# Boese0601/MagicDance

Hardware: NVIDIA H100
Metric: denoise-steps/sec @512x512 50-step DDIM (higher is better)
Workload: dtype f16

## Files before the change

### magicdance_b200/csrc/attention.cu

```cuda
#include <stdlib.h>

#include <type_traits>

#include "common.cuh"

namespace mdb {

constexpr int kBQ = 128;

template <int D, int BKV, int STAGES>
struct AttnCfg {
  static constexpr int kDkChunks = (D + 63) / 64;
  static constexpr int kDV = (D + 15) / 16 * 16;
  static constexpr int kKSteps = kDV / 16;
  static constexpr int kQBytes = kDkChunks * kBQ * 128;
  static constexpr int kKBytes = kDkChunks * BKV * 128;
  static constexpr int kVBytes = kDV * 128;
  static constexpr int kStageBytes = kKBytes + kVBytes;
  static constexpr int kSmem = kQBytes + STAGES * kStageBytes + 1024;
  static_assert(BKV == 64, "one 128-byte swizzle row of keys per V^T tile");
  static_assert(kVBytes % 1024 == 0 && kKBytes % 1024 == 0, "stage tiles start on swizzle-atom boundaries");
};

struct AttnKParams {
  CUtensorMap tmQ, tmK0, tmV0, tmK1, tmV1;
  __half* out;
  long long ldo;
  int nq, n0, n1;
  int kv0_batches, kv1_batches;
  int bank_batches;
  float scale_log2;
};
struct AttnLseKParams : AttnKParams {
  float* lse;
};

template <int D, int BKV, int STAGES, int MINB, bool LSE = false>
__global__ void __launch_bounds__(kWsThreads, MINB)
    attn_wg_kernel(const __grid_constant__ std::conditional_t<LSE, AttnLseKParams, AttnKParams> p) {
  using C = AttnCfg<D, BKV, STAGES>;
  extern __shared__ uint8_t smem_raw[];
  __shared__ __align__(8) uint64_t q_bar;
  __shared__ __align__(8) uint64_t kv_full[STAGES], kv_empty[STAGES];

  uint8_t* sQ = align1024(smem_raw);
  uint8_t* sKV = sQ + C::kQBytes;

  const int warp = threadIdx.x >> 5;
  const int lane = threadIdx.x & 31;
  const int q0 = blockIdx.x * kBQ;
  const int head = blockIdx.y;
  const int b = blockIdx.z;
  const int t0 = (p.n0 + BKV - 1) / BKV;
  const int t1 = (b < p.bank_batches && p.n1 > 0) ? (p.n1 + BKV - 1) / BKV : 0;
  const int n_tiles = t0 + t1;

  pdl_launch_dependents();
  if (warp == kProducerWarp && lane == 0) {
    tma_prefetch_desc(&p.tmQ);
    tma_prefetch_desc(&p.tmK0);
    tma_prefetch_desc(&p.tmV0);
    mbar_init(&q_bar, 1);
    ring_init<STAGES>(kv_full, kv_empty, 1);
    fence_barrier_init();
  }
  __syncthreads();
  pdl_wait();

  if (warp == kProducerWarp) {
    if (lane == 0) {
      mbar_expect_tx(&q_bar, C::kQBytes);
      for (int dc = 0; dc < C::kDkChunks; ++dc)
        tma_load_3d(sQ + dc * (kBQ * 128), &p.tmQ, &q_bar, dc * 64, head, b * p.nq + q0);
      for (int j = 0; j < n_tiles; ++j) {
        const bool src1 = j >= t0;
        const int key0 = (src1 ? (j - t0) : j) * BKV;
        const CUtensorMap* tk = src1 ? &p.tmK1 : &p.tmK0;
        const CUtensorMap* tv = src1 ? &p.tmV1 : &p.tmV0;
        const int nsrc = src1 ? p.n1 : p.n0;
        const int kvb = src1 ? (p.kv1_batches > 1 ? b : 0) : (p.kv0_batches > 1 ? b : 0);
        const int s = ring_acquire<STAGES>(kv_empty, j);
        mbar_expect_tx(&kv_full[s], C::kStageBytes);
        uint8_t* sk = sKV + s * C::kStageBytes;
        uint8_t* sv = sk + C::kKBytes;
        for (int dc = 0; dc < C::kDkChunks; ++dc)
          tma_load_3d(sk + dc * (BKV * 128), tk, &kv_full[s], dc * 64, head, kvb * nsrc + key0);
        tma_load_3d(sv, tv, &kv_full[s], key0, kvb, head * D);
      }
    }
  } else {
    const int wg = warp >> 2;
    const uint32_t q_addr = smem_u32(sQ) + wg * (64 * 128);
    const int cq = 2 * (lane & 3);
    float o[C::kDV / 2];
#pragma unroll
    for (int i = 0; i < C::kDV / 2; ++i) o[i] = 0.f;
    float m_run[2] = {-INFINITY, -INFINITY};
    float l_run[2] = {0.f, 0.f};
    mbar_wait(&q_bar, 0);

    for (int j = 0; j < n_tiles; ++j) {
      const bool src1 = j >= t0;
      const int key0 = (src1 ? (j - t0) : j) * BKV;
      const int valid = min(BKV, (src1 ? p.n1 : p.n0) - key0);
      const int s = ring_wait_full<STAGES>(kv_full, j);
      const uint32_t k_addr = smem_u32(sKV + s * C::kStageBytes);
      const uint32_t v_addr = k_addr + C::kKBytes;

      float sc[BKV / 2];
      wgmma_fence();
#pragma unroll
      for (int ks = 0; ks < C::kKSteps; ++ks) {
        const int dc = ks >> 2, kk = ks & 3;
        const uint64_t da = wgmma_desc_k_sw128(q_addr + dc * (kBQ * 128)) + 2 * kk;
        const uint64_t db = wgmma_desc_k_sw128(k_addr + dc * (BKV * 128)) + 2 * kk;
        wgmma_ss<BKV>(sc, da, db, ks != 0 ? 1u : 0u);
      }
      wgmma_commit();
      wgmma_wait<0>();
      wgmma_fence_regs(sc);

      if (valid < BKV) {
#pragma unroll
        for (int i = 0; i < BKV / 2; ++i)
          if (8 * (i >> 2) + cq + (i & 1) >= valid) sc[i] = -INFINITY;
      }
      float mx[2] = {-INFINITY, -INFINITY};
#pragma unroll
      for (int i = 0; i < BKV / 2; ++i) mx[(i >> 1) & 1] = fmaxf(mx[(i >> 1) & 1], sc[i]);
      float alpha[2], neg_m[2];
#pragma unroll
      for (int h = 0; h < 2; ++h) {
        mx[h] = fmaxf(mx[h], __shfl_xor_sync(0xffffffffu, mx[h], 1));
        mx[h] = fmaxf(mx[h], __shfl_xor_sync(0xffffffffu, mx[h], 2));
        const float m_new = fmaxf(m_run[h], mx[h] * p.scale_log2);
        alpha[h] = ex2_approx(m_run[h] - m_new);
        m_run[h] = m_new;
        neg_m[h] = -m_new;
      }
      float ls[2] = {0.f, 0.f};
      uint32_t pa[BKV / 16][4];
#pragma unroll
      for (int i = 0; i < BKV / 2; i += 2) {
        const int h = (i >> 1) & 1;
        const float e0 = ex2_approx(fmaf(sc[i], p.scale_log2, neg_m[h]));
        const float e1 = ex2_approx(fmaf(sc[i + 1], p.scale_log2, neg_m[h]));
        ls[h] += e0 + e1;
        pa[i >> 3][(i >> 1) & 3] = pack_half2(e0, e1);
      }
#pragma unroll
      for (int h = 0; h < 2; ++h) l_run[h] = fmaf(l_run[h], alpha[h], ls[h]);
#pragma unroll
      for (int i = 0; i < C::kDV / 2; ++i) o[i] *= alpha[(i >> 1) & 1];

      wgmma_fence();
#pragma unroll
      for (int kk = 0; kk < BKV / 16; ++kk)
        wgmma_rs<C::kDV>(o, pa[kk], wgmma_desc_k_sw128(v_addr) + 2 * kk, 1u);
      wgmma_commit();
      wgmma_wait<0>();
      wgmma_fence_regs(o);
      mbar_arrive(&kv_empty[s]);
    }

    float inv_l[2], l_row[2];
#pragma unroll
    for (int h = 0; h < 2; ++h) {
      float l = l_run[h];
      l += __shfl_xor_sync(0xffffffffu, l, 1);
      l += __shfl_xor_sync(0xffffffffu, l, 2);
      inv_l[h] = 1.0f / l;
      l_row[h] = l;
    }
    const int r = wg * 64 + (warp & 3) * 16 + (lane >> 2);
    if constexpr (LSE) {
      if ((lane & 3) == 0) {
#pragma unroll
        for (int h = 0; h < 2; ++h) {
          const int q = q0 + r + 8 * h;
          if (q < p.nq)
            p.lse[(static_cast<long long>(b) * gridDim.y + head) * p.nq + q] =
                (m_run[h] + log2f(l_row[h])) * 0.6931471805599453f;
        }
      }
    }
#pragma unroll
    for (int h = 0; h < 2; ++h) {
      const int q = q0 + r + 8 * h;
      if (q < p.nq) {
        __half* op = p.out + (static_cast<long long>(b) * p.nq + q) * p.ldo + head * D + cq;
#pragma unroll
        for (int c8 = 0; c8 < D / 8; ++c8)
          *reinterpret_cast<uint32_t*>(op + 8 * c8) =
              pack_half2(o[4 * c8 + 2 * h] * inv_l[h], o[4 * c8 + 2 * h + 1] * inv_l[h]);
      }
    }
  }
}

static int g_attn40_2q_min_ctas = 512;
int get_attn_tuning() { return g_attn40_2q_min_ctas; }
void set_attn_tuning(int v) { g_attn40_2q_min_ctas = v; }

template <int D, int BKV, int STAGES, int MINB, bool LSE = false, typename P>
static int launch_attn(const P& kp, dim3 grid, cudaStream_t st) {
  using C = AttnCfg<D, BKV, STAGES>;
  static_assert(MINB == 1 || C::kSmem <= 113 * 1024, "two CTAs per SM must fit");
  constexpr auto kern = attn_wg_kernel<D, BKV, STAGES, MINB, LSE>;
  if (int rc = set_max_dyn_smem<kern>(C::kSmem)) return rc;
  MDB_CHECK_CUDA(launch_pdl(kern, grid, dim3(kWsThreads), C::kSmem, st, kp));
  count_launch();
  return MDB_OK;
}

template <int D, int BKV>
static int build_and_launch(const mdb_attn_desc* a, float* lse, cudaStream_t st) {
  constexpr int kDV = AttnCfg<D, BKV, 1>::kDV;
  AttnKParams kp;
  memset(&kp, 0, sizeof(kp));
  const int hd = a->heads * a->d;
  int rc;
  if ((rc = tmap_heads(&kp.tmQ, a->q, a->d, a->heads, (uint64_t)a->batch * a->nq, a->ldq, kBQ))) return rc;
  auto mk_kv = [&](const void* k, long long ldk, const void* vt, long long ldvt, int n, int nb, int ldvb,
                   CUtensorMap* tk, CUtensorMap* tv) -> int {
    int r = tmap_heads(tk, k, a->d, a->heads, (uint64_t)nb * n, ldk, BKV);
    if (r) return r;
    return tmap_vt(tv, vt, n, nb, ldvb, hd, ldvt, kDV);
  };
  if ((rc = mk_kv(a->k0, a->ldk0, a->vt0, a->ldvt0, a->n0, a->kv0_batches, a->ldv0_batch, &kp.tmK0, &kp.tmV0))) return rc;
  if (a->n1 > 0) {
    if ((rc = mk_kv(a->k1, a->ldk1, a->vt1, a->ldvt1, a->n1, a->kv1_batches, a->ldv1_batch, &kp.tmK1, &kp.tmV1)))
      return rc;
  }
  kp.out = static_cast<__half*>(a->out);
  kp.ldo = a->ldo;
  kp.nq = a->nq;
  kp.n0 = a->n0;
  kp.n1 = a->n1;
  kp.kv0_batches = a->kv0_batches;
  kp.kv1_batches = a->kv1_batches;
  kp.bank_batches = a->n1 > 0 ? a->bank_batches : 0;
  kp.scale_log2 = a->scale * 1.4426950408889634f;
  dim3 grid((a->nq + kBQ - 1) / kBQ, a->heads, a->batch);
  if (lse != nullptr) {
    AttnLseKParams lp;
    memset(&lp, 0, sizeof(lp));
    static_cast<AttnKParams&>(lp) = kp;
    lp.lse = lse;
    if constexpr (D == 40) {
      const long long ctas = (long long)grid.x * grid.y * grid.z;
      if (ctas >= (long long)g_attn40_2q_min_ctas) return launch_attn<D, BKV, 3, 2, true>(lp, grid, st);
    }
    return launch_attn<D, BKV, (D == 160 ? 2 : 4), 1, true>(lp, grid, st);
  }
  if constexpr (D == 40) {
    const long long ctas = (long long)grid.x * grid.y * grid.z;
    if (ctas >= (long long)g_attn40_2q_min_ctas) return launch_attn<D, BKV, 3, 2>(kp, grid, st);
  }
  return launch_attn<D, BKV, (D == 160 ? 2 : 4), 1>(kp, grid, st);
}

static int attention_entry(const mdb_attn_desc* a, float* lse, cudaStream_t st) {
  switch (a->d) {
    case 40:
      return build_and_launch<40, 64>(a, lse, st);
    case 80:
      return build_and_launch<80, 64>(a, lse, st);
    case 160:
      return build_and_launch<160, 64>(a, lse, st);
    default:
      set_error("mdb_attention_f16: head dim %d not supported (40, 80, 160)", a->d);
      return MDB_ERR_UNSUPPORTED;
  }
}

int attention_check_desc(const mdb_attn_desc* a) {
  MDB_REQUIRE(a != nullptr, "mdb_attention_f16: null descriptor");
  MDB_REQUIRE(a->q && a->k0 && a->vt0 && a->out, "mdb_attention_f16: null operand");
  MDB_REQUIRE(a->batch > 0 && a->heads > 0 && a->nq > 0 && a->n0 > 0 && a->n1 >= 0,
              "mdb_attention_f16: bad shape");
  MDB_REQUIRE(a->n1 == 0 || (a->k1 && a->vt1), "mdb_attention_f16: n1 > 0 needs k1/vt1");
  MDB_REQUIRE(a->kv0_batches == 1 || a->kv0_batches == a->batch, "mdb_attention_f16: kv0_batches must be 1 or batch");
  MDB_REQUIRE(a->n1 == 0 || a->kv1_batches == 1 || a->kv1_batches >= a->bank_batches,
              "mdb_attention_f16: kv1_batches must be 1 or cover bank_batches");
  MDB_REQUIRE(a->ldv0_batch >= a->n0 && a->ldv0_batch % 8 == 0, "mdb_attention_f16: ldv0_batch must be >= n0 and %% 8");
  MDB_REQUIRE(a->n1 == 0 || (a->ldv1_batch >= a->n1 && a->ldv1_batch % 8 == 0),
              "mdb_attention_f16: ldv1_batch must be >= n1 and %% 8");
  MDB_REQUIRE(a->ldo % 8 == 0 && (reinterpret_cast<uintptr_t>(a->out) & 15) == 0, "mdb_attention_f16: out alignment");
  return MDB_OK;
}

}

using namespace mdb;

extern "C" int mdb_attention_f16(const mdb_attn_desc* a, mdb_stream_t stream) {
  const int rc = attention_check_desc(a);
  if (rc) return rc;
  return attention_entry(a, nullptr, static_cast<cudaStream_t>(stream));
}

extern "C" int mdb_attention_lse_f16(const mdb_attn_desc* a, float* lse, mdb_stream_t stream) {
  const int rc = attention_check_desc(a);
  if (rc) return rc;
  MDB_REQUIRE(lse != nullptr, "mdb_attention_lse_f16: null lse");
  return attention_entry(a, lse, static_cast<cudaStream_t>(stream));
}
```

### magicdance_b200/csrc/wgmma.cuh

```cuda
#pragma once
#include <stdint.h>

namespace mdb {

template <int N, int TA = 0, int TB = 0>
__device__ __forceinline__ void wgmma_ss(float (&d)[N / 2], uint64_t da, uint64_t db, uint32_t acc);
template <int N, int TB = 0>
__device__ __forceinline__ void wgmma_rs(float (&d)[N / 2], const uint32_t (&a)[4], uint64_t db, uint32_t acc);

template <>
__device__ __forceinline__ void wgmma_ss<64, 0, 0>(float (&d)[32], uint64_t da, uint64_t db, uint32_t acc) {
  asm volatile(
      "{\n\t.reg .pred p;\n\tsetp.ne.b32 p, %34, 0;\n\t"
      "wgmma.mma_async.sync.aligned.m64n64k16.f32.f16.f16 {%0, %1, %2, %3, %4, %5, %6, %7, %8, %9, %10, %11, %12, %13, %14, %15, %16, %17, %18, %19, %20, %21, %22, %23, %24, %25, %26, %27, %28, %29, %30, %31}, %32, %33, p, 1, 1, 0, 0;\n\t}"
      : "+f"(d[0]), "+f"(d[1]), "+f"(d[2]), "+f"(d[3]), "+f"(d[4]), "+f"(d[5]), "+f"(d[6]), "+f"(d[7]), "+f"(d[8]), "+f"(d[9]), "+f"(d[10]), "+f"(d[11]), "+f"(d[12]), "+f"(d[13]), "+f"(d[14]), "+f"(d[15]), "+f"(d[16]), "+f"(d[17]), "+f"(d[18]), "+f"(d[19]), "+f"(d[20]), "+f"(d[21]), "+f"(d[22]), "+f"(d[23]), "+f"(d[24]), "+f"(d[25]), "+f"(d[26]), "+f"(d[27]), "+f"(d[28]), "+f"(d[29]), "+f"(d[30]), "+f"(d[31])
      : "l"(da), "l"(db), "r"(acc));
}

template <>
__device__ __forceinline__ void wgmma_ss<80, 0, 0>(float (&d)[40], uint64_t da, uint64_t db, uint32_t acc) {
  asm volatile(
      "{\n\t.reg .pred p;\n\tsetp.ne.b32 p, %42, 0;\n\t"
      "wgmma.mma_async.sync.aligned.m64n80k16.f32.f16.f16 {%0, %1, %2, %3, %4, %5, %6, %7, %8, %9, %10, %11, %12, %13, %14, %15, %16, %17, %18, %19, %20, %21, %22, %23, %24, %25, %26, %27, %28, %29, %30, %31, %32, %33, %34, %35, %36, %37, %38, %39}, %40, %41, p, 1, 1, 0, 0;\n\t}"
      : "+f"(d[0]), "+f"(d[1]), "+f"(d[2]), "+f"(d[3]), "+f"(d[4]), "+f"(d[5]), "+f"(d[6]), "+f"(d[7]), "+f"(d[8]), "+f"(d[9]), "+f"(d[10]), "+f"(d[11]), "+f"(d[12]), "+f"(d[13]), "+f"(d[14]), "+f"(d[15]), "+f"(d[16]), "+f"(d[17]), "+f"(d[18]), "+f"(d[19]), "+f"(d[20]), "+f"(d[21]), "+f"(d[22]), "+f"(d[23]), "+f"(d[24]), "+f"(d[25]), "+f"(d[26]), "+f"(d[27]), "+f"(d[28]), "+f"(d[29]), "+f"(d[30]), "+f"(d[31]), "+f"(d[32]), "+f"(d[33]), "+f"(d[34]), "+f"(d[35]), "+f"(d[36]), "+f"(d[37]), "+f"(d[38]), "+f"(d[39])
      : "l"(da), "l"(db), "r"(acc));
}

template <>
__device__ __forceinline__ void wgmma_ss<128, 0, 0>(float (&d)[64], uint64_t da, uint64_t db, uint32_t acc) {
  asm volatile(
      "{\n\t.reg .pred p;\n\tsetp.ne.b32 p, %66, 0;\n\t"
      "wgmma.mma_async.sync.aligned.m64n128k16.f32.f16.f16 {%0, %1, %2, %3, %4, %5, %6, %7, %8, %9, %10, %11, %12, %13, %14, %15, %16, %17, %18, %19, %20, %21, %22, %23, %24, %25, %26, %27, %28, %29, %30, %31, %32, %33, %34, %35, %36, %37, %38, %39, %40, %41, %42, %43, %44, %45, %46, %47, %48, %49, %50, %51, %52, %53, %54, %55, %56, %57, %58, %59, %60, %61, %62, %63}, %64, %65, p, 1, 1, 0, 0;\n\t}"
      : "+f"(d[0]), "+f"(d[1]), "+f"(d[2]), "+f"(d[3]), "+f"(d[4]), "+f"(d[5]), "+f"(d[6]), "+f"(d[7]), "+f"(d[8]), "+f"(d[9]), "+f"(d[10]), "+f"(d[11]), "+f"(d[12]), "+f"(d[13]), "+f"(d[14]), "+f"(d[15]), "+f"(d[16]), "+f"(d[17]), "+f"(d[18]), "+f"(d[19]), "+f"(d[20]), "+f"(d[21]), "+f"(d[22]), "+f"(d[23]), "+f"(d[24]), "+f"(d[25]), "+f"(d[26]), "+f"(d[27]), "+f"(d[28]), "+f"(d[29]), "+f"(d[30]), "+f"(d[31]), "+f"(d[32]), "+f"(d[33]), "+f"(d[34]), "+f"(d[35]), "+f"(d[36]), "+f"(d[37]), "+f"(d[38]), "+f"(d[39]), "+f"(d[40]), "+f"(d[41]), "+f"(d[42]), "+f"(d[43]), "+f"(d[44]), "+f"(d[45]), "+f"(d[46]), "+f"(d[47]), "+f"(d[48]), "+f"(d[49]), "+f"(d[50]), "+f"(d[51]), "+f"(d[52]), "+f"(d[53]), "+f"(d[54]), "+f"(d[55]), "+f"(d[56]), "+f"(d[57]), "+f"(d[58]), "+f"(d[59]), "+f"(d[60]), "+f"(d[61]), "+f"(d[62]), "+f"(d[63])
      : "l"(da), "l"(db), "r"(acc));
}

template <>
__device__ __forceinline__ void wgmma_ss<160, 0, 0>(float (&d)[80], uint64_t da, uint64_t db, uint32_t acc) {
  asm volatile(
      "{\n\t.reg .pred p;\n\tsetp.ne.b32 p, %82, 0;\n\t"
      "wgmma.mma_async.sync.aligned.m64n160k16.f32.f16.f16 {%0, %1, %2, %3, %4, %5, %6, %7, %8, %9, %10, %11, %12, %13, %14, %15, %16, %17, %18, %19, %20, %21, %22, %23, %24, %25, %26, %27, %28, %29, %30, %31, %32, %33, %34, %35, %36, %37, %38, %39, %40, %41, %42, %43, %44, %45, %46, %47, %48, %49, %50, %51, %52, %53, %54, %55, %56, %57, %58, %59, %60, %61, %62, %63, %64, %65, %66, %67, %68, %69, %70, %71, %72, %73, %74, %75, %76, %77, %78, %79}, %80, %81, p, 1, 1, 0, 0;\n\t}"
      : "+f"(d[0]), "+f"(d[1]), "+f"(d[2]), "+f"(d[3]), "+f"(d[4]), "+f"(d[5]), "+f"(d[6]), "+f"(d[7]), "+f"(d[8]), "+f"(d[9]), "+f"(d[10]), "+f"(d[11]), "+f"(d[12]), "+f"(d[13]), "+f"(d[14]), "+f"(d[15]), "+f"(d[16]), "+f"(d[17]), "+f"(d[18]), "+f"(d[19]), "+f"(d[20]), "+f"(d[21]), "+f"(d[22]), "+f"(d[23]), "+f"(d[24]), "+f"(d[25]), "+f"(d[26]), "+f"(d[27]), "+f"(d[28]), "+f"(d[29]), "+f"(d[30]), "+f"(d[31]), "+f"(d[32]), "+f"(d[33]), "+f"(d[34]), "+f"(d[35]), "+f"(d[36]), "+f"(d[37]), "+f"(d[38]), "+f"(d[39]), "+f"(d[40]), "+f"(d[41]), "+f"(d[42]), "+f"(d[43]), "+f"(d[44]), "+f"(d[45]), "+f"(d[46]), "+f"(d[47]), "+f"(d[48]), "+f"(d[49]), "+f"(d[50]), "+f"(d[51]), "+f"(d[52]), "+f"(d[53]), "+f"(d[54]), "+f"(d[55]), "+f"(d[56]), "+f"(d[57]), "+f"(d[58]), "+f"(d[59]), "+f"(d[60]), "+f"(d[61]), "+f"(d[62]), "+f"(d[63]), "+f"(d[64]), "+f"(d[65]), "+f"(d[66]), "+f"(d[67]), "+f"(d[68]), "+f"(d[69]), "+f"(d[70]), "+f"(d[71]), "+f"(d[72]), "+f"(d[73]), "+f"(d[74]), "+f"(d[75]), "+f"(d[76]), "+f"(d[77]), "+f"(d[78]), "+f"(d[79])
      : "l"(da), "l"(db), "r"(acc));
}

template <>
__device__ __forceinline__ void wgmma_ss<256, 0, 0>(float (&d)[128], uint64_t da, uint64_t db, uint32_t acc) {
  asm volatile(
      "{\n\t.reg .pred p;\n\tsetp.ne.b32 p, %130, 0;\n\t"
      "wgmma.mma_async.sync.aligned.m64n256k16.f32.f16.f16 {%0, %1, %2, %3, %4, %5, %6, %7, %8, %9, %10, %11, %12, %13, %14, %15, %16, %17, %18, %19, %20, %21, %22, %23, %24, %25, %26, %27, %28, %29, %30, %31, %32, %33, %34, %35, %36, %37, %38, %39, %40, %41, %42, %43, %44, %45, %46, %47, %48, %49, %50, %51, %52, %53, %54, %55, %56, %57, %58, %59, %60, %61, %62, %63, %64, %65, %66, %67, %68, %69, %70, %71, %72, %73, %74, %75, %76, %77, %78, %79, %80, %81, %82, %83, %84, %85, %86, %87, %88, %89, %90, %91, %92, %93, %94, %95, %96, %97, %98, %99, %100, %101, %102, %103, %104, %105, %106, %107, %108, %109, %110, %111, %112, %113, %114, %115, %116, %117, %118, %119, %120, %121, %122, %123, %124, %125, %126, %127}, %128, %129, p, 1, 1, 0, 0;\n\t}"
      : "+f"(d[0]), "+f"(d[1]), "+f"(d[2]), "+f"(d[3]), "+f"(d[4]), "+f"(d[5]), "+f"(d[6]), "+f"(d[7]), "+f"(d[8]), "+f"(d[9]), "+f"(d[10]), "+f"(d[11]), "+f"(d[12]), "+f"(d[13]), "+f"(d[14]), "+f"(d[15]), "+f"(d[16]), "+f"(d[17]), "+f"(d[18]), "+f"(d[19]), "+f"(d[20]), "+f"(d[21]), "+f"(d[22]), "+f"(d[23]), "+f"(d[24]), "+f"(d[25]), "+f"(d[26]), "+f"(d[27]), "+f"(d[28]), "+f"(d[29]), "+f"(d[30]), "+f"(d[31]), "+f"(d[32]), "+f"(d[33]), "+f"(d[34]), "+f"(d[35]), "+f"(d[36]), "+f"(d[37]), "+f"(d[38]), "+f"(d[39]), "+f"(d[40]), "+f"(d[41]), "+f"(d[42]), "+f"(d[43]), "+f"(d[44]), "+f"(d[45]), "+f"(d[46]), "+f"(d[47]), "+f"(d[48]), "+f"(d[49]), "+f"(d[50]), "+f"(d[51]), "+f"(d[52]), "+f"(d[53]), "+f"(d[54]), "+f"(d[55]), "+f"(d[56]), "+f"(d[57]), "+f"(d[58]), "+f"(d[59]), "+f"(d[60]), "+f"(d[61]), "+f"(d[62]), "+f"(d[63]), "+f"(d[64]), "+f"(d[65]), "+f"(d[66]), "+f"(d[67]), "+f"(d[68]), "+f"(d[69]), "+f"(d[70]), "+f"(d[71]), "+f"(d[72]), "+f"(d[73]), "+f"(d[74]), "+f"(d[75]), "+f"(d[76]), "+f"(d[77]), "+f"(d[78]), "+f"(d[79]), "+f"(d[80]), "+f"(d[81]), "+f"(d[82]), "+f"(d[83]), "+f"(d[84]), "+f"(d[85]), "+f"(d[86]), "+f"(d[87]), "+f"(d[88]), "+f"(d[89]), "+f"(d[90]), "+f"(d[91]), "+f"(d[92]), "+f"(d[93]), "+f"(d[94]), "+f"(d[95]), "+f"(d[96]), "+f"(d[97]), "+f"(d[98]), "+f"(d[99]), "+f"(d[100]), "+f"(d[101]), "+f"(d[102]), "+f"(d[103]), "+f"(d[104]), "+f"(d[105]), "+f"(d[106]), "+f"(d[107]), "+f"(d[108]), "+f"(d[109]), "+f"(d[110]), "+f"(d[111]), "+f"(d[112]), "+f"(d[113]), "+f"(d[114]), "+f"(d[115]), "+f"(d[116]), "+f"(d[117]), "+f"(d[118]), "+f"(d[119]), "+f"(d[120]), "+f"(d[121]), "+f"(d[122]), "+f"(d[123]), "+f"(d[124]), "+f"(d[125]), "+f"(d[126]), "+f"(d[127])
      : "l"(da), "l"(db), "r"(acc));
}

template <>
__device__ __forceinline__ void wgmma_ss<64, 0, 1>(float (&d)[32], uint64_t da, uint64_t db, uint32_t acc) {
  asm volatile(
      "{\n\t.reg .pred p;\n\tsetp.ne.b32 p, %34, 0;\n\t"
      "wgmma.mma_async.sync.aligned.m64n64k16.f32.f16.f16 {%0, %1, %2, %3, %4, %5, %6, %7, %8, %9, %10, %11, %12, %13, %14, %15, %16, %17, %18, %19, %20, %21, %22, %23, %24, %25, %26, %27, %28, %29, %30, %31}, %32, %33, p, 1, 1, 0, 1;\n\t}"
      : "+f"(d[0]), "+f"(d[1]), "+f"(d[2]), "+f"(d[3]), "+f"(d[4]), "+f"(d[5]), "+f"(d[6]), "+f"(d[7]), "+f"(d[8]), "+f"(d[9]), "+f"(d[10]), "+f"(d[11]), "+f"(d[12]), "+f"(d[13]), "+f"(d[14]), "+f"(d[15]), "+f"(d[16]), "+f"(d[17]), "+f"(d[18]), "+f"(d[19]), "+f"(d[20]), "+f"(d[21]), "+f"(d[22]), "+f"(d[23]), "+f"(d[24]), "+f"(d[25]), "+f"(d[26]), "+f"(d[27]), "+f"(d[28]), "+f"(d[29]), "+f"(d[30]), "+f"(d[31])
      : "l"(da), "l"(db), "r"(acc));
}

template <>
__device__ __forceinline__ void wgmma_ss<64, 1, 0>(float (&d)[32], uint64_t da, uint64_t db, uint32_t acc) {
  asm volatile(
      "{\n\t.reg .pred p;\n\tsetp.ne.b32 p, %34, 0;\n\t"
      "wgmma.mma_async.sync.aligned.m64n64k16.f32.f16.f16 {%0, %1, %2, %3, %4, %5, %6, %7, %8, %9, %10, %11, %12, %13, %14, %15, %16, %17, %18, %19, %20, %21, %22, %23, %24, %25, %26, %27, %28, %29, %30, %31}, %32, %33, p, 1, 1, 1, 0;\n\t}"
      : "+f"(d[0]), "+f"(d[1]), "+f"(d[2]), "+f"(d[3]), "+f"(d[4]), "+f"(d[5]), "+f"(d[6]), "+f"(d[7]), "+f"(d[8]), "+f"(d[9]), "+f"(d[10]), "+f"(d[11]), "+f"(d[12]), "+f"(d[13]), "+f"(d[14]), "+f"(d[15]), "+f"(d[16]), "+f"(d[17]), "+f"(d[18]), "+f"(d[19]), "+f"(d[20]), "+f"(d[21]), "+f"(d[22]), "+f"(d[23]), "+f"(d[24]), "+f"(d[25]), "+f"(d[26]), "+f"(d[27]), "+f"(d[28]), "+f"(d[29]), "+f"(d[30]), "+f"(d[31])
      : "l"(da), "l"(db), "r"(acc));
}

template <>
__device__ __forceinline__ void wgmma_ss<128, 0, 1>(float (&d)[64], uint64_t da, uint64_t db, uint32_t acc) {
  asm volatile(
      "{\n\t.reg .pred p;\n\tsetp.ne.b32 p, %66, 0;\n\t"
      "wgmma.mma_async.sync.aligned.m64n128k16.f32.f16.f16 {%0, %1, %2, %3, %4, %5, %6, %7, %8, %9, %10, %11, %12, %13, %14, %15, %16, %17, %18, %19, %20, %21, %22, %23, %24, %25, %26, %27, %28, %29, %30, %31, %32, %33, %34, %35, %36, %37, %38, %39, %40, %41, %42, %43, %44, %45, %46, %47, %48, %49, %50, %51, %52, %53, %54, %55, %56, %57, %58, %59, %60, %61, %62, %63}, %64, %65, p, 1, 1, 0, 1;\n\t}"
      : "+f"(d[0]), "+f"(d[1]), "+f"(d[2]), "+f"(d[3]), "+f"(d[4]), "+f"(d[5]), "+f"(d[6]), "+f"(d[7]), "+f"(d[8]), "+f"(d[9]), "+f"(d[10]), "+f"(d[11]), "+f"(d[12]), "+f"(d[13]), "+f"(d[14]), "+f"(d[15]), "+f"(d[16]), "+f"(d[17]), "+f"(d[18]), "+f"(d[19]), "+f"(d[20]), "+f"(d[21]), "+f"(d[22]), "+f"(d[23]), "+f"(d[24]), "+f"(d[25]), "+f"(d[26]), "+f"(d[27]), "+f"(d[28]), "+f"(d[29]), "+f"(d[30]), "+f"(d[31]), "+f"(d[32]), "+f"(d[33]), "+f"(d[34]), "+f"(d[35]), "+f"(d[36]), "+f"(d[37]), "+f"(d[38]), "+f"(d[39]), "+f"(d[40]), "+f"(d[41]), "+f"(d[42]), "+f"(d[43]), "+f"(d[44]), "+f"(d[45]), "+f"(d[46]), "+f"(d[47]), "+f"(d[48]), "+f"(d[49]), "+f"(d[50]), "+f"(d[51]), "+f"(d[52]), "+f"(d[53]), "+f"(d[54]), "+f"(d[55]), "+f"(d[56]), "+f"(d[57]), "+f"(d[58]), "+f"(d[59]), "+f"(d[60]), "+f"(d[61]), "+f"(d[62]), "+f"(d[63])
      : "l"(da), "l"(db), "r"(acc));
}

template <>
__device__ __forceinline__ void wgmma_ss<128, 1, 1>(float (&d)[64], uint64_t da, uint64_t db, uint32_t acc) {
  asm volatile(
      "{\n\t.reg .pred p;\n\tsetp.ne.b32 p, %66, 0;\n\t"
      "wgmma.mma_async.sync.aligned.m64n128k16.f32.f16.f16 {%0, %1, %2, %3, %4, %5, %6, %7, %8, %9, %10, %11, %12, %13, %14, %15, %16, %17, %18, %19, %20, %21, %22, %23, %24, %25, %26, %27, %28, %29, %30, %31, %32, %33, %34, %35, %36, %37, %38, %39, %40, %41, %42, %43, %44, %45, %46, %47, %48, %49, %50, %51, %52, %53, %54, %55, %56, %57, %58, %59, %60, %61, %62, %63}, %64, %65, p, 1, 1, 1, 1;\n\t}"
      : "+f"(d[0]), "+f"(d[1]), "+f"(d[2]), "+f"(d[3]), "+f"(d[4]), "+f"(d[5]), "+f"(d[6]), "+f"(d[7]), "+f"(d[8]), "+f"(d[9]), "+f"(d[10]), "+f"(d[11]), "+f"(d[12]), "+f"(d[13]), "+f"(d[14]), "+f"(d[15]), "+f"(d[16]), "+f"(d[17]), "+f"(d[18]), "+f"(d[19]), "+f"(d[20]), "+f"(d[21]), "+f"(d[22]), "+f"(d[23]), "+f"(d[24]), "+f"(d[25]), "+f"(d[26]), "+f"(d[27]), "+f"(d[28]), "+f"(d[29]), "+f"(d[30]), "+f"(d[31]), "+f"(d[32]), "+f"(d[33]), "+f"(d[34]), "+f"(d[35]), "+f"(d[36]), "+f"(d[37]), "+f"(d[38]), "+f"(d[39]), "+f"(d[40]), "+f"(d[41]), "+f"(d[42]), "+f"(d[43]), "+f"(d[44]), "+f"(d[45]), "+f"(d[46]), "+f"(d[47]), "+f"(d[48]), "+f"(d[49]), "+f"(d[50]), "+f"(d[51]), "+f"(d[52]), "+f"(d[53]), "+f"(d[54]), "+f"(d[55]), "+f"(d[56]), "+f"(d[57]), "+f"(d[58]), "+f"(d[59]), "+f"(d[60]), "+f"(d[61]), "+f"(d[62]), "+f"(d[63])
      : "l"(da), "l"(db), "r"(acc));
}

template <>
__device__ __forceinline__ void wgmma_rs<48, 0>(float (&d)[24], const uint32_t (&a)[4], uint64_t db, uint32_t acc) {
  asm volatile(
      "{\n\t.reg .pred p;\n\tsetp.ne.b32 p, %29, 0;\n\t"
      "wgmma.mma_async.sync.aligned.m64n48k16.f32.f16.f16 {%0, %1, %2, %3, %4, %5, %6, %7, %8, %9, %10, %11, %12, %13, %14, %15, %16, %17, %18, %19, %20, %21, %22, %23}, {%24, %25, %26, %27}, %28, p, 1, 1, 0;\n\t}"
      : "+f"(d[0]), "+f"(d[1]), "+f"(d[2]), "+f"(d[3]), "+f"(d[4]), "+f"(d[5]), "+f"(d[6]), "+f"(d[7]), "+f"(d[8]), "+f"(d[9]), "+f"(d[10]), "+f"(d[11]), "+f"(d[12]), "+f"(d[13]), "+f"(d[14]), "+f"(d[15]), "+f"(d[16]), "+f"(d[17]), "+f"(d[18]), "+f"(d[19]), "+f"(d[20]), "+f"(d[21]), "+f"(d[22]), "+f"(d[23])
      : "r"(a[0]), "r"(a[1]), "r"(a[2]), "r"(a[3]), "l"(db), "r"(acc));
}

template <>
__device__ __forceinline__ void wgmma_rs<80, 0>(float (&d)[40], const uint32_t (&a)[4], uint64_t db, uint32_t acc) {
  asm volatile(
      "{\n\t.reg .pred p;\n\tsetp.ne.b32 p, %45, 0;\n\t"
      "wgmma.mma_async.sync.aligned.m64n80k16.f32.f16.f16 {%0, %1, %2, %3, %4, %5, %6, %7, %8, %9, %10, %11, %12, %13, %14, %15, %16, %17, %18, %19, %20, %21, %22, %23, %24, %25, %26, %27, %28, %29, %30, %31, %32, %33, %34, %35, %36, %37, %38, %39}, {%40, %41, %42, %43}, %44, p, 1, 1, 0;\n\t}"
      : "+f"(d[0]), "+f"(d[1]), "+f"(d[2]), "+f"(d[3]), "+f"(d[4]), "+f"(d[5]), "+f"(d[6]), "+f"(d[7]), "+f"(d[8]), "+f"(d[9]), "+f"(d[10]), "+f"(d[11]), "+f"(d[12]), "+f"(d[13]), "+f"(d[14]), "+f"(d[15]), "+f"(d[16]), "+f"(d[17]), "+f"(d[18]), "+f"(d[19]), "+f"(d[20]), "+f"(d[21]), "+f"(d[22]), "+f"(d[23]), "+f"(d[24]), "+f"(d[25]), "+f"(d[26]), "+f"(d[27]), "+f"(d[28]), "+f"(d[29]), "+f"(d[30]), "+f"(d[31]), "+f"(d[32]), "+f"(d[33]), "+f"(d[34]), "+f"(d[35]), "+f"(d[36]), "+f"(d[37]), "+f"(d[38]), "+f"(d[39])
      : "r"(a[0]), "r"(a[1]), "r"(a[2]), "r"(a[3]), "l"(db), "r"(acc));
}

template <>
__device__ __forceinline__ void wgmma_rs<160, 0>(float (&d)[80], const uint32_t (&a)[4], uint64_t db, uint32_t acc) {
  asm volatile(
      "{\n\t.reg .pred p;\n\tsetp.ne.b32 p, %85, 0;\n\t"
      "wgmma.mma_async.sync.aligned.m64n160k16.f32.f16.f16 {%0, %1, %2, %3, %4, %5, %6, %7, %8, %9, %10, %11, %12, %13, %14, %15, %16, %17, %18, %19, %20, %21, %22, %23, %24, %25, %26, %27, %28, %29, %30, %31, %32, %33, %34, %35, %36, %37, %38, %39, %40, %41, %42, %43, %44, %45, %46, %47, %48, %49, %50, %51, %52, %53, %54, %55, %56, %57, %58, %59, %60, %61, %62, %63, %64, %65, %66, %67, %68, %69, %70, %71, %72, %73, %74, %75, %76, %77, %78, %79}, {%80, %81, %82, %83}, %84, p, 1, 1, 0;\n\t}"
      : "+f"(d[0]), "+f"(d[1]), "+f"(d[2]), "+f"(d[3]), "+f"(d[4]), "+f"(d[5]), "+f"(d[6]), "+f"(d[7]), "+f"(d[8]), "+f"(d[9]), "+f"(d[10]), "+f"(d[11]), "+f"(d[12]), "+f"(d[13]), "+f"(d[14]), "+f"(d[15]), "+f"(d[16]), "+f"(d[17]), "+f"(d[18]), "+f"(d[19]), "+f"(d[20]), "+f"(d[21]), "+f"(d[22]), "+f"(d[23]), "+f"(d[24]), "+f"(d[25]), "+f"(d[26]), "+f"(d[27]), "+f"(d[28]), "+f"(d[29]), "+f"(d[30]), "+f"(d[31]), "+f"(d[32]), "+f"(d[33]), "+f"(d[34]), "+f"(d[35]), "+f"(d[36]), "+f"(d[37]), "+f"(d[38]), "+f"(d[39]), "+f"(d[40]), "+f"(d[41]), "+f"(d[42]), "+f"(d[43]), "+f"(d[44]), "+f"(d[45]), "+f"(d[46]), "+f"(d[47]), "+f"(d[48]), "+f"(d[49]), "+f"(d[50]), "+f"(d[51]), "+f"(d[52]), "+f"(d[53]), "+f"(d[54]), "+f"(d[55]), "+f"(d[56]), "+f"(d[57]), "+f"(d[58]), "+f"(d[59]), "+f"(d[60]), "+f"(d[61]), "+f"(d[62]), "+f"(d[63]), "+f"(d[64]), "+f"(d[65]), "+f"(d[66]), "+f"(d[67]), "+f"(d[68]), "+f"(d[69]), "+f"(d[70]), "+f"(d[71]), "+f"(d[72]), "+f"(d[73]), "+f"(d[74]), "+f"(d[75]), "+f"(d[76]), "+f"(d[77]), "+f"(d[78]), "+f"(d[79])
      : "r"(a[0]), "r"(a[1]), "r"(a[2]), "r"(a[3]), "l"(db), "r"(acc));
}

template <>
__device__ __forceinline__ void wgmma_rs<48, 1>(float (&d)[24], const uint32_t (&a)[4], uint64_t db, uint32_t acc) {
  asm volatile(
      "{\n\t.reg .pred p;\n\tsetp.ne.b32 p, %29, 0;\n\t"
      "wgmma.mma_async.sync.aligned.m64n48k16.f32.f16.f16 {%0, %1, %2, %3, %4, %5, %6, %7, %8, %9, %10, %11, %12, %13, %14, %15, %16, %17, %18, %19, %20, %21, %22, %23}, {%24, %25, %26, %27}, %28, p, 1, 1, 1;\n\t}"
      : "+f"(d[0]), "+f"(d[1]), "+f"(d[2]), "+f"(d[3]), "+f"(d[4]), "+f"(d[5]), "+f"(d[6]), "+f"(d[7]), "+f"(d[8]), "+f"(d[9]), "+f"(d[10]), "+f"(d[11]), "+f"(d[12]), "+f"(d[13]), "+f"(d[14]), "+f"(d[15]), "+f"(d[16]), "+f"(d[17]), "+f"(d[18]), "+f"(d[19]), "+f"(d[20]), "+f"(d[21]), "+f"(d[22]), "+f"(d[23])
      : "r"(a[0]), "r"(a[1]), "r"(a[2]), "r"(a[3]), "l"(db), "r"(acc));
}

template <>
__device__ __forceinline__ void wgmma_rs<80, 1>(float (&d)[40], const uint32_t (&a)[4], uint64_t db, uint32_t acc) {
  asm volatile(
      "{\n\t.reg .pred p;\n\tsetp.ne.b32 p, %45, 0;\n\t"
      "wgmma.mma_async.sync.aligned.m64n80k16.f32.f16.f16 {%0, %1, %2, %3, %4, %5, %6, %7, %8, %9, %10, %11, %12, %13, %14, %15, %16, %17, %18, %19, %20, %21, %22, %23, %24, %25, %26, %27, %28, %29, %30, %31, %32, %33, %34, %35, %36, %37, %38, %39}, {%40, %41, %42, %43}, %44, p, 1, 1, 1;\n\t}"
      : "+f"(d[0]), "+f"(d[1]), "+f"(d[2]), "+f"(d[3]), "+f"(d[4]), "+f"(d[5]), "+f"(d[6]), "+f"(d[7]), "+f"(d[8]), "+f"(d[9]), "+f"(d[10]), "+f"(d[11]), "+f"(d[12]), "+f"(d[13]), "+f"(d[14]), "+f"(d[15]), "+f"(d[16]), "+f"(d[17]), "+f"(d[18]), "+f"(d[19]), "+f"(d[20]), "+f"(d[21]), "+f"(d[22]), "+f"(d[23]), "+f"(d[24]), "+f"(d[25]), "+f"(d[26]), "+f"(d[27]), "+f"(d[28]), "+f"(d[29]), "+f"(d[30]), "+f"(d[31]), "+f"(d[32]), "+f"(d[33]), "+f"(d[34]), "+f"(d[35]), "+f"(d[36]), "+f"(d[37]), "+f"(d[38]), "+f"(d[39])
      : "r"(a[0]), "r"(a[1]), "r"(a[2]), "r"(a[3]), "l"(db), "r"(acc));
}

template <>
__device__ __forceinline__ void wgmma_rs<160, 1>(float (&d)[80], const uint32_t (&a)[4], uint64_t db, uint32_t acc) {
  asm volatile(
      "{\n\t.reg .pred p;\n\tsetp.ne.b32 p, %85, 0;\n\t"
      "wgmma.mma_async.sync.aligned.m64n160k16.f32.f16.f16 {%0, %1, %2, %3, %4, %5, %6, %7, %8, %9, %10, %11, %12, %13, %14, %15, %16, %17, %18, %19, %20, %21, %22, %23, %24, %25, %26, %27, %28, %29, %30, %31, %32, %33, %34, %35, %36, %37, %38, %39, %40, %41, %42, %43, %44, %45, %46, %47, %48, %49, %50, %51, %52, %53, %54, %55, %56, %57, %58, %59, %60, %61, %62, %63, %64, %65, %66, %67, %68, %69, %70, %71, %72, %73, %74, %75, %76, %77, %78, %79}, {%80, %81, %82, %83}, %84, p, 1, 1, 1;\n\t}"
      : "+f"(d[0]), "+f"(d[1]), "+f"(d[2]), "+f"(d[3]), "+f"(d[4]), "+f"(d[5]), "+f"(d[6]), "+f"(d[7]), "+f"(d[8]), "+f"(d[9]), "+f"(d[10]), "+f"(d[11]), "+f"(d[12]), "+f"(d[13]), "+f"(d[14]), "+f"(d[15]), "+f"(d[16]), "+f"(d[17]), "+f"(d[18]), "+f"(d[19]), "+f"(d[20]), "+f"(d[21]), "+f"(d[22]), "+f"(d[23]), "+f"(d[24]), "+f"(d[25]), "+f"(d[26]), "+f"(d[27]), "+f"(d[28]), "+f"(d[29]), "+f"(d[30]), "+f"(d[31]), "+f"(d[32]), "+f"(d[33]), "+f"(d[34]), "+f"(d[35]), "+f"(d[36]), "+f"(d[37]), "+f"(d[38]), "+f"(d[39]), "+f"(d[40]), "+f"(d[41]), "+f"(d[42]), "+f"(d[43]), "+f"(d[44]), "+f"(d[45]), "+f"(d[46]), "+f"(d[47]), "+f"(d[48]), "+f"(d[49]), "+f"(d[50]), "+f"(d[51]), "+f"(d[52]), "+f"(d[53]), "+f"(d[54]), "+f"(d[55]), "+f"(d[56]), "+f"(d[57]), "+f"(d[58]), "+f"(d[59]), "+f"(d[60]), "+f"(d[61]), "+f"(d[62]), "+f"(d[63]), "+f"(d[64]), "+f"(d[65]), "+f"(d[66]), "+f"(d[67]), "+f"(d[68]), "+f"(d[69]), "+f"(d[70]), "+f"(d[71]), "+f"(d[72]), "+f"(d[73]), "+f"(d[74]), "+f"(d[75]), "+f"(d[76]), "+f"(d[77]), "+f"(d[78]), "+f"(d[79])
      : "r"(a[0]), "r"(a[1]), "r"(a[2]), "r"(a[3]), "l"(db), "r"(acc));
}

}
```

Measured before the change: 89.85.

## Overlap next-tile QK wgmma with current PV wgmma and softmax in attention

Restructures the attention consumer loop into a software pipeline. The QK^T wgmma for the next KV tile is issued together with the PV wgmma for the current tile, and softmax on the new scores runs while PV is still in flight. This hides tensor-core latency behind softmax math. It also narrows the PV N dimension to a multiple of 8 (adding an m64n40 instruction for D=40), which drops padded columns. The pipelined path is enabled for all head sizes except 160, and it keeps more registers live per thread.

```diff
diff --git a/magicdance_b200/csrc/attention.cu b/magicdance_b200/csrc/attention.cu
--- a/magicdance_b200/csrc/attention.cu
+++ b/magicdance_b200/csrc/attention.cu
@@ -12,6 +12,7 @@
 struct AttnCfg {
   static constexpr int kDkChunks = (D + 63) / 64;
   static constexpr int kDV = (D + 15) / 16 * 16;
+  static constexpr int kPvN = (D + 7) / 8 * 8;
   static constexpr int kKSteps = kDV / 16;
   static constexpr int kQBytes = kDkChunks * kBQ * 128;
   static constexpr int kKBytes = kDkChunks * BKV * 128;
@@ -35,7 +36,71 @@
   float* lse;
 };
 
-template <int D, int BKV, int STAGES, int MINB, bool LSE = false>
+template <int D, int BKV>
+__device__ __forceinline__ void attn_issue_qk(float (&sc)[BKV / 2], uint32_t q_addr, uint32_t k_addr) {
+  using C = AttnCfg<D, BKV, 1>;
+  wgmma_fence();
+#pragma unroll
+  for (int ks = 0; ks < C::kKSteps; ++ks) {
+    const int dc = ks >> 2, kk = ks & 3;
+    const uint64_t da = wgmma_desc_k_sw128(q_addr + dc * (kBQ * 128)) + 2 * kk;
+    const uint64_t db = wgmma_desc_k_sw128(k_addr + dc * (BKV * 128)) + 2 * kk;
+    wgmma_ss<BKV>(sc, da, db, ks != 0 ? 1u : 0u);
+  }
+  wgmma_commit();
+}
+
+template <int BKV>
+__device__ __forceinline__ void attn_softmax(float (&sc)[BKV / 2], int valid, float scale_log2, float (&m_run)[2],
+                                             float (&l_run)[2], float (&alpha)[2]) {
+  const int cq = 2 * (threadIdx.x & 3);
+  if (valid < BKV) {
+#pragma unroll
+    for (int i = 0; i < BKV / 2; ++i)
+      if (8 * (i >> 2) + cq + (i & 1) >= valid) sc[i] = -INFINITY;
+  }
+  float mx[2] = {-INFINITY, -INFINITY};
+#pragma unroll
+  for (int i = 0; i < BKV / 2; ++i) mx[(i >> 1) & 1] = fmaxf(mx[(i >> 1) & 1], sc[i]);
+  float neg_m[2];
+#pragma unroll
+  for (int h = 0; h < 2; ++h) {
+    mx[h] = fmaxf(mx[h], __shfl_xor_sync(0xffffffffu, mx[h], 1));
+    mx[h] = fmaxf(mx[h], __shfl_xor_sync(0xffffffffu, mx[h], 2));
+    const float m_new = fmaxf(m_run[h], mx[h] * scale_log2);
+    alpha[h] = ex2_approx(m_run[h] - m_new);
+    m_run[h] = m_new;
+    neg_m[h] = -m_new;
+  }
+  float ls[2] = {0.f, 0.f};
+#pragma unroll
+  for (int i = 0; i < BKV / 2; i += 2) {
+    const int h = (i >> 1) & 1;
+    sc[i] = ex2_approx(fmaf(sc[i], scale_log2, neg_m[h]));
+    sc[i + 1] = ex2_approx(fmaf(sc[i + 1], scale_log2, neg_m[h]));
+    ls[h] += sc[i] + sc[i + 1];
+  }
+#pragma unroll
+  for (int h = 0; h < 2; ++h) l_run[h] = fmaf(l_run[h], alpha[h], ls[h]);
+}
+
+template <int BKV>
+__device__ __forceinline__ void attn_pack_p(const float (&sc)[BKV / 2], uint32_t (&pa)[BKV / 16][4]) {
+#pragma unroll
+  for (int i = 0; i < BKV / 2; i += 2) pa[i >> 3][(i >> 1) & 3] = pack_half2(sc[i], sc[i + 1]);
+}
+
+template <int D, int BKV>
+__device__ __forceinline__ void attn_issue_pv(float (&o)[AttnCfg<D, BKV, 1>::kPvN / 2],
+                                              const uint32_t (&pa)[BKV / 16][4], uint32_t v_addr) {
+  wgmma_fence();
+#pragma unroll
+  for (int kk = 0; kk < BKV / 16; ++kk)
+    wgmma_rs<AttnCfg<D, BKV, 1>::kPvN>(o, pa[kk], wgmma_desc_k_sw128(v_addr) + 2 * kk, 1u);
+  wgmma_commit();
+}
+
+template <int D, int BKV, int STAGES, int MINB, bool PIPE, bool LSE = false>
 __global__ void __launch_bounds__(kWsThreads, MINB)
     attn_wg_kernel(const __grid_constant__ std::conditional_t<LSE, AttnLseKParams, AttnKParams> p) {
   using C = AttnCfg<D, BKV, STAGES>;
@@ -92,75 +157,63 @@
     const int wg = warp >> 2;
     const uint32_t q_addr = smem_u32(sQ) + wg * (64 * 128);
     const int cq = 2 * (lane & 3);
-    float o[C::kDV / 2];
-#pragma unroll
-    for (int i = 0; i < C::kDV / 2; ++i) o[i] = 0.f;
+    float o[C::kPvN / 2];
+#pragma unroll
+    for (int i = 0; i < C::kPvN / 2; ++i) o[i] = 0.f;
     float m_run[2] = {-INFINITY, -INFINITY};
     float l_run[2] = {0.f, 0.f};
     mbar_wait(&q_bar, 0);
 
-    for (int j = 0; j < n_tiles; ++j) {
+    auto tile_valid = [&](int j) {
       const bool src1 = j >= t0;
-      const int key0 = (src1 ? (j - t0) : j) * BKV;
-      const int valid = min(BKV, (src1 ? p.n1 : p.n0) - key0);
-      const int s = ring_wait_full<STAGES>(kv_full, j);
-      const uint32_t k_addr = smem_u32(sKV + s * C::kStageBytes);
-      const uint32_t v_addr = k_addr + C::kKBytes;
-
-      float sc[BKV / 2];
-      wgmma_fence();
-#pragma unroll
-      for (int ks = 0; ks < C::kKSteps; ++ks) {
-        const int dc = ks >> 2, kk = ks & 3;
-        const uint64_t da = wgmma_desc_k_sw128(q_addr + dc * (kBQ * 128)) + 2 * kk;
-        const uint64_t db = wgmma_desc_k_sw128(k_addr + dc * (BKV * 128)) + 2 * kk;
-        wgmma_ss<BKV>(sc, da, db, ks != 0 ? 1u : 0u);
-      }
-      wgmma_commit();
+      return min(BKV, (src1 ? p.n1 : p.n0) - (src1 ? (j - t0) : j) * BKV);
+    };
+    auto tile_k = [&](int j) { return smem_u32(sKV + ring_wait_full<STAGES>(kv_full, j) * C::kStageBytes); };
+
+    float sc[BKV / 2];
+    uint32_t pa[BKV / 16][4];
+    float alpha[2];
+    if constexpr (!PIPE) {
+      for (int j = 0; j < n_tiles; ++j) {
+        const uint32_t k_addr = tile_k(j);
+        attn_issue_qk<D, BKV>(sc, q_addr, k_addr);
+        wgmma_wait<0>();
+        wgmma_fence_regs(sc);
+        attn_softmax<BKV>(sc, tile_valid(j), p.scale_log2, m_run, l_run, alpha);
+        attn_pack_p<BKV>(sc, pa);
+#pragma unroll
+        for (int i = 0; i < C::kPvN / 2; ++i) o[i] *= alpha[(i >> 1) & 1];
+        attn_issue_pv<D, BKV>(o, pa, k_addr + C::kKBytes);
+        wgmma_wait<0>();
+        wgmma_fence_regs(o);
+        mbar_arrive(&kv_empty[j % STAGES]);
+      }
+    } else {
+      uint32_t k_addr = tile_k(0);
+      attn_issue_qk<D, BKV>(sc, q_addr, k_addr);
       wgmma_wait<0>();
       wgmma_fence_regs(sc);
-
-      if (valid < BKV) {
-#pragma unroll
-        for (int i = 0; i < BKV / 2; ++i)
-          if (8 * (i >> 2) + cq + (i & 1) >= valid) sc[i] = -INFINITY;
-      }
-      float mx[2] = {-INFINITY, -INFINITY};
-#pragma unroll
-      for (int i = 0; i < BKV / 2; ++i) mx[(i >> 1) & 1] = fmaxf(mx[(i >> 1) & 1], sc[i]);
-      float alpha[2], neg_m[2];
-#pragma unroll
-      for (int h = 0; h < 2; ++h) {
-        mx[h] = fmaxf(mx[h], __shfl_xor_sync(0xffffffffu, mx[h], 1));
-        mx[h] = fmaxf(mx[h], __shfl_xor_sync(0xffffffffu, mx[h], 2));
-        const float m_new = fmaxf(m_run[h], mx[h] * p.scale_log2);
-        alpha[h] = ex2_approx(m_run[h] - m_new);
-        m_run[h] = m_new;
-        neg_m[h] = -m_new;
-      }
-      float ls[2] = {0.f, 0.f};
-      uint32_t pa[BKV / 16][4];
-#pragma unroll
-      for (int i = 0; i < BKV / 2; i += 2) {
-        const int h = (i >> 1) & 1;
-        const float e0 = ex2_approx(fmaf(sc[i], p.scale_log2, neg_m[h]));
-        const float e1 = ex2_approx(fmaf(sc[i + 1], p.scale_log2, neg_m[h]));
-        ls[h] += e0 + e1;
-        pa[i >> 3][(i >> 1) & 3] = pack_half2(e0, e1);
-      }
-#pragma unroll
-      for (int h = 0; h < 2; ++h) l_run[h] = fmaf(l_run[h], alpha[h], ls[h]);
-#pragma unroll
-      for (int i = 0; i < C::kDV / 2; ++i) o[i] *= alpha[(i >> 1) & 1];
-
-      wgmma_fence();
-#pragma unroll
-      for (int kk = 0; kk < BKV / 16; ++kk)
-        wgmma_rs<C::kDV>(o, pa[kk], wgmma_desc_k_sw128(v_addr) + 2 * kk, 1u);
-      wgmma_commit();
+      attn_softmax<BKV>(sc, tile_valid(0), p.scale_log2, m_run, l_run, alpha);
+      attn_pack_p<BKV>(sc, pa);
+      for (int j = 0; j + 1 < n_tiles; ++j) {
+        const uint32_t v_addr = k_addr + C::kKBytes;
+        k_addr = tile_k(j + 1);
+        attn_issue_qk<D, BKV>(sc, q_addr, k_addr);
+        attn_issue_pv<D, BKV>(o, pa, v_addr);
+        wgmma_wait<1>();
+        wgmma_fence_regs(sc);
+        attn_softmax<BKV>(sc, tile_valid(j + 1), p.scale_log2, m_run, l_run, alpha);
+        wgmma_wait<0>();
+        wgmma_fence_regs(o);
+        mbar_arrive(&kv_empty[j % STAGES]);
+#pragma unroll
+        for (int i = 0; i < C::kPvN / 2; ++i) o[i] *= alpha[(i >> 1) & 1];
+        attn_pack_p<BKV>(sc, pa);
+      }
+      attn_issue_pv<D, BKV>(o, pa, k_addr + C::kKBytes);
       wgmma_wait<0>();
       wgmma_fence_regs(o);
-      mbar_arrive(&kv_empty[s]);
+      mbar_arrive(&kv_empty[(n_tiles - 1) % STAGES]);
     }
 
     float inv_l[2], l_row[2];
@@ -202,15 +255,24 @@
 int get_attn_tuning() { return g_attn40_2q_min_ctas; }
 void set_attn_tuning(int v) { g_attn40_2q_min_ctas = v; }
 
-template <int D, int BKV, int STAGES, int MINB, bool LSE = false, typename P>
+template <int D, int BKV, int STAGES, int MINB, bool PIPE, bool LSE, typename P>
 static int launch_attn(const P& kp, dim3 grid, cudaStream_t st) {
   using C = AttnCfg<D, BKV, STAGES>;
   static_assert(MINB == 1 || C::kSmem <= 113 * 1024, "two CTAs per SM must fit");
-  constexpr auto kern = attn_wg_kernel<D, BKV, STAGES, MINB, LSE>;
+  constexpr auto kern = attn_wg_kernel<D, BKV, STAGES, MINB, PIPE, LSE>;
   if (int rc = set_max_dyn_smem<kern>(C::kSmem)) return rc;
   MDB_CHECK_CUDA(launch_pdl(kern, grid, dim3(kWsThreads), C::kSmem, st, kp));
   count_launch();
   return MDB_OK;
+}
+
+template <int D, int BKV, bool LSE, typename P>
+static int launch_for_grid(const P& kp, dim3 grid, cudaStream_t st) {
+  if constexpr (D == 40) {
+    const long long ctas = (long long)grid.x * grid.y * grid.z;
+    if (ctas >= (long long)g_attn40_2q_min_ctas) return launch_attn<D, BKV, 3, 2, true, LSE>(kp, grid, st);
+  }
+  return launch_attn<D, BKV, (D == 160 ? 2 : 4), 1, D != 160, LSE>(kp, grid, st);
 }
 
 template <int D, int BKV>
@@ -247,17 +309,9 @@
     memset(&lp, 0, sizeof(lp));
     static_cast<AttnKParams&>(lp) = kp;
     lp.lse = lse;
-    if constexpr (D == 40) {
-      const long long ctas = (long long)grid.x * grid.y * grid.z;
-      if (ctas >= (long long)g_attn40_2q_min_ctas) return launch_attn<D, BKV, 3, 2, true>(lp, grid, st);
-    }
-    return launch_attn<D, BKV, (D == 160 ? 2 : 4), 1, true>(lp, grid, st);
-  }
-  if constexpr (D == 40) {
-    const long long ctas = (long long)grid.x * grid.y * grid.z;
-    if (ctas >= (long long)g_attn40_2q_min_ctas) return launch_attn<D, BKV, 3, 2>(kp, grid, st);
-  }
-  return launch_attn<D, BKV, (D == 160 ? 2 : 4), 1>(kp, grid, st);
+    return launch_for_grid<D, BKV, true>(lp, grid, st);
+  }
+  return launch_for_grid<D, BKV, false>(kp, grid, st);
 }
 
 static int attention_entry(const mdb_attn_desc* a, float* lse, cudaStream_t st) {
diff --git a/magicdance_b200/csrc/wgmma.cuh b/magicdance_b200/csrc/wgmma.cuh
--- a/magicdance_b200/csrc/wgmma.cuh
+++ b/magicdance_b200/csrc/wgmma.cuh
@@ -90,6 +90,15 @@
 }
 
 template <>
+__device__ __forceinline__ void wgmma_rs<40, 0>(float (&d)[20], const uint32_t (&a)[4], uint64_t db, uint32_t acc) {
+  asm volatile(
+      "{\n\t.reg .pred p;\n\tsetp.ne.b32 p, %25, 0;\n\t"
+      "wgmma.mma_async.sync.aligned.m64n40k16.f32.f16.f16 {%0, %1, %2, %3, %4, %5, %6, %7, %8, %9, %10, %11, %12, %13, %14, %15, %16, %17, %18, %19}, {%20, %21, %22, %23}, %24, p, 1, 1, 0;\n\t}"
+      : "+f"(d[0]), "+f"(d[1]), "+f"(d[2]), "+f"(d[3]), "+f"(d[4]), "+f"(d[5]), "+f"(d[6]), "+f"(d[7]), "+f"(d[8]), "+f"(d[9]), "+f"(d[10]), "+f"(d[11]), "+f"(d[12]), "+f"(d[13]), "+f"(d[14]), "+f"(d[15]), "+f"(d[16]), "+f"(d[17]), "+f"(d[18]), "+f"(d[19])
+      : "r"(a[0]), "r"(a[1]), "r"(a[2]), "r"(a[3]), "l"(db), "r"(acc));
+}
+
+template <>
 __device__ __forceinline__ void wgmma_rs<48, 0>(float (&d)[24], const uint32_t (&a)[4], uint64_t db, uint32_t acc) {
   asm volatile(
       "{\n\t.reg .pred p;\n\tsetp.ne.b32 p, %29, 0;\n\t"
```

After: 90.96, median of 6. 1.2% higher.
